# jchibane/Box2Mask

Hardware: AMD Instinct MI355X
Metric: ScanNet scenes/sec (fwd+bwd, ~150k voxels @2cm) (higher is better)
Workload: dtype f32; 1 GPU; ScanNet 2cm voxels, batch_size=8 per GPU, sparse-conv fwd/bwd + losses + Adam (BASELINE configs[1]); global_batch=8, ranks_seen=1, voxels_per_gpu_batch=1202778, parallelism=dp1, distinct_batches=4, setup_steps=2, prefetch=next batch: coordinate + kernel maps on a second stream during the step, steps_executed=51, full=False

## Files before the change

box2mask_amd/_lib.py:

```python
from __future__ import annotations

import ctypes as C
import os

import torch

_HERE = os.path.dirname(os.path.abspath(__file__))
LIB_PATH = os.environ.get('B2M_LIB_PATH', os.path.join(_HERE, 'libb2m_hip.so'))

P = C.c_void_p
I32 = C.c_int32
I64 = C.c_int64
F32 = C.c_float
F64 = C.c_double

PROTOTYPES = {
    'b2m_coords_build': [P, I64, P, P, I64, P, P],
    'b2m_morton_keys': [P, I64, P, P],
    'b2m_hilbert_keys': [P, I64, I32, P, P],
    'b2m_coords_stride': [P, I64, I32, P, P, P, P, P, I64, P, C.POINTER(I64), P],
    'b2m_kernel_map': [P, I64, I32, I32, P, P, I64, P, I32, I32, I32, P, I64, P],
    'b2m_occupancy': [P, I64, I32, I32, I32, I32, P, I64, P],
    'b2m_kernel_map_rulebook': [P, I64, I32, I32, P, P, I64, P, I32, I32, I32, P, P, P, P],
    'b2m_stride_tables': [P, P, I64, I64, P, I64, P, I64, P],
    'b2m_rulebook': [P, I64, I32, I64, P, P, P, P, P],
    'b2m_rulebook_balance': [P, I32, I64, P],
    'b2m_detection_loss': [P, I64, P, I64, P, I64, P, I64, I32, P, P, P, P, P, I64, F64, P, F32, F32, F32, F32, F32, P, P, P, P, P, P, P, P],
    'b2m_radix_argsort': [P, I64, C.c_uint64, P, P, P, P],
    'b2m_conv_fwd': [P, I64, I32, P, I64, I32, I64, P, I32, P, P, P, P, I64, P, I64, I32, I32, P],
    'b2m_conv_fwd_affine': [P, I64, I32, P, I64, I32, I64, P, I32, P, P, P, I64, P, I64, I32, P, P, P, I64, I32, P, P],
    'b2m_conv_fwd_h': [P, I64, I32, P, I64, I32, I64, P, I32, P, P, P, I64, P, I64, I32, P, P, P, I64, I32, P],
    'b2m_conv_fwd_h_stats': [P, I64, I32, P, I64, I32, I64, P, I32, P, P, P, I64, P, I64, I32, P, P],
    'b2m_weight_pack_h': [P, I64, I32, I32, I32, I32, P, P],
    'b2m_conv_fwd_stats': [P, I64, I32, P, I64, I32, I64, P, I32, P, P, P, P, I64, P, I64, I32, I32, P, P, P],
    'b2m_conv_wgrad_h': [P, I64, I32, I64, P, I64, I32, P, P, P, I64, I32, P, I64, I64, I32, F32, P],
    'b2m_weight_pack_h_t': [P, I32, I32, I32, I32, I32, I32, P, P],
    'b2m_bn_stats_finalize_h': [P, I64, I64, I32, P, P, P, F32, F32, P, P, P, P, P, P, P],
    'b2m_bn_stats_h': [P, I64, I64, I32, P, P, P],
    'b2m_bn_apply_h': [P, I64, I64, I32, P, P, P, I64, I32, P, I64, P],
    'b2m_bn_bwd_reduce_h': [P, I64, P, I64, P, I64, I64, I32, P, P, I32, P, P, P, P, P, P, F32, P],
    'b2m_bn_bwd_apply_h': [P, I64, P, I64, P, I64, I64, I32, P, P, P, P, F64, P, I32, P, P, P, I64, P, I64, P],
    'b2m_half_absmax': [P, I64, I64, I32, P, P],
    'b2m_f32_absmax': [P, I64, P, P],
    'b2m_guard_finish': [P, P, P, P],
    'b2m_clock_probe': [P, I32, P],
    'b2m_xchg_allreduce': [P, I32, P, I32, I32, C.c_uint64, P, P, P],
    'b2m_conv_up': [P, I64, I32, P, I64, I32, I64, P, I32, P, P, P, P, P, I64, I32, I64, I32, P, P, P, I64, I32, P, P],
    'b2m_weight_pack': [P, I64, I32, I32, I32, I32, I32, I32, I32, P, P],
    'b2m_weight_pack_run': [P, I32, I64, P],
    'b2m_weight_pack_h_run': [P, I32, I64, P],
    'b2m_conv_wgrad': [P, I64, I32, I64, P, I64, I32, P, P, P, I64, I32, P, I64, I64, P, P],
    'b2m_conv_wgrad_tr': [P, I64, I32, I64, P, I64, I32, P, P, P, I64, I32, P, I64, I64, P, P],
    'b2m_bn_stats': [P, I64, I64, I32, P, P, P],
    'b2m_bn_tilestats': [P, I64, I32, P, P, P],
    'b2m_bn_tilestats_finalize': [P, I64, I64, I32, P, P, P, P, F32, F32, P, P, P, P, P, P, P],
    'b2m_bn_finalize': [P, F64, P, I32, P, P, F32, F32, P, P, P, P, P, P, P],
    'b2m_bn_apply': [P, I64, I64, I32, P, P, P, I64, I32, P, I64, P],
    'b2m_bn_bwd_reduce': [P, I64, P, I64, P, I64, I64, I32, P, P, I32, P, P, P, P, P, P, P],
    'b2m_bn_stats_finalize': [P, I64, I64, I32, P, P, P, P, F32, F32, P, P, P, P, P, P, P],
    'b2m_bn_bwd_apply': [P, I64, P, I64, P, I64, I64, I32, P, P, P, P, F64, P, I32, P, P, P, I64, P, I64, P],
    'b2m_bn_apply2': [P, I64, P, I64, I64, I32, P, P, P, P, I32, P, I64, P],
    'b2m_bn_bwd_reduce2': [P, I64, P, I64, P, I64, P, I64, I64, I32, P, P, P, P, I32, P, P, P],
    'b2m_bn_bwd_apply2': [P, I64, P, I64, P, I64, P, I64, I64, I32, P, P, P, P, P, P, P, F64, P, I32, P, I64, P, I64, P, P, P, P, P, P],
    'b2m_bn_small_fwd': [P, I64, I64, I32, P, P, F32, F32, P, P, P, P, P, P, P, I64, I32, P, I64, P],
    'b2m_bn_small_fwd_stats': [P, I64, I64, I32, P, P],
    'b2m_bn_small_fwd_apply': [P, P, I64, I64, I32, P, P, F32, F32, P, P, P, P, P, P, P, I64, I32, P, I64, P],
    'b2m_bn_small_bwd_phase': [I32, P, I64, P, I64, P, I64, I64, I32, P, P, P, I32, P, P, P, P, P, I64, P, I64, P, P, P],
    'b2m_bn_small_bwd': [P, I64, P, I64, P, I64, I64, I32, P, P, P, I32, P, P, P, P, P, I64, P, I64, P],
    'b2m_relu_fwd': [P, I64, P, P],
    'b2m_relu_bwd': [P, P, I64, P, P],
    'b2m_add': [P, P, I64, P, P],
    'b2m_segment_pool_fwd': [P, I64, I64, I32, P, I64, I32, P, P, P, P, P],
    'b2m_segment_mean_sorted': [P, I64, I64, I32, P, P, I64, P, P, P],
    'b2m_segment_pool_bwd': [P, I64, I32, P, I64, I32, P, P, P, I64, P],
    'b2m_nmc': [P, I32, F32, I32, P, P, P, P, P, P],
    'b2m_nmc_batch': [P, P, I32, I32, F32, P, P, P, P, P, P],
    'b2m_mask_project': [P, I32, P, I32, P, P, I64, F32, P, I64, P],
    'b2m_mask_nms': [P, I32, I64, F32, P, P, P, P],
    'b2m_label_hist': [P, I64, P, I32, P, I64, I32, P, P],
    'b2m_mask_gather': [P, I64, P, I32, P, I64, P, P],
    'b2m_mask_project_batch': [P, I32, I64, I64, F32, P],
    'b2m_mask_nms_batch': [P, I32, I32, F32, P],
    'b2m_label_hist_batch': [P, I32, I64, I32, P],
    'b2m_mask_gather_batch': [P, I32, I64, I64, P],
    'b2m_mask_gather_batch_t': [P, I32, I64, I64, I64, P, P],
    'b2m_mask_nms_sweep': [P, I32, I64, P, I32, P, P, P],
    'b2m_mask_nms_sweep_batch': [P, I32, I32, P, I32, P, I64, P],
    'b2m_mask_hist_index': [P, I64, I32, I64, P, P, I64, I32, P, P, P],
    'b2m_mask_hist_index_batch': [P, I32, I64, I64, P],
    'b2m_mask_hist': [P, I64, I32, P, I64, I32, P, P],
    'b2m_mask_pack': [P, I32, I64, P, I64, P],
    'b2m_set_ious': [P, P, I64, P, P],
    'b2m_mask_hulls': [P, I64, I32, P, I64, P, P, P, I32, P, P, P, P, P, P, P],
    'b2m_mask_hulls_index': [P, I64, I32, I64, P, P, I64, P, P, P, P, I32, P, P, P, P, P, P, P],
    'b2m_mask_hulls_index_batch': [P, I32, I32, I32, I64, P],
    'b2m_obb_corners': [P, P, P, I32, P, P],
    'b2m_hull_box_iou': [P, P, P, P, I32, P, P, I32, P, P],
    'b2m_aabb_iou': [P, P, I32, P, P, P, I32, P, P],
    'b2m_dbscan': [P, I64, I32, F64, I32, P, P, P, P],
    'b2m_paint_proposals': [P, I64, I32, P, I64, I32, F64, I32, P, P, P, P, P],
    'b2m_joint_hist': [P, P, I64, I32, I32, P, P],
    'b2m_vox_shift': [P, I64, P, P, P],
    'b2m_unique_insert_async': [P, I64, P, I64, P, P, P, P],
    'b2m_vox_keys': [P, I64, P, F64, P, P, P],
    'b2m_sort_u64': [P, I64, P],
    'b2m_unique_rank': [P, I64, P, P, I64, P, I64, P, P],
    'b2m_vox_decode': [P, I64, I32, P, P],
    'b2m_vox_nearest': [P, I64, P, F64, P, P, I64, I64, P, P, P],
    'b2m_vox_gather': [P, I64, P, P, P, P, P, P],
    'b2m_seg_centroid': [P, P, I64, I64, F64, P, P, P, P, P],
    'b2m_box_membership': [P, I64, P, P, P, I32, P, P, P, P],
    'b2m_seg_box_vote': [P, I64, P, P, I64, I64, P, P, P, P, I32, P, P, P, P, P],
    'b2m_obb_membership': [P, I64, P, P, P, I32, P, P, P],
# ... 123 lines not shown
```

box2mask_amd/csrc/conv.hip:

```cpp
#include "b2m_common.h"
#include <stdlib.h>
#include <type_traits>

struct ConvArgs {
    const float* x1; int64_t ldx1; int c1;
    const float* x2; int64_t ldx2; int c2;
    const float* wp; int K;
    const float* bias;
    const int32_t* rb_in; const uint8_t* rb_out; const int32_t* rb_cnt;
    int64_t n_out, ntiles;
    float* y; int64_t ldy; int cout; int accumulate; int nstrips; int vec_store;
    int nslice;
    int chain;
    int fast32;
    const float* zeros;
    int ncs;
    int wg_combine;
    int64_t nwg;
    int64_t xcd_per;
    const int32_t* xcd_start;
    int64_t wg_per_tile;
    const int32_t* tile_order;
    double* stats;
    const float* ep_scale; const float* ep_shift; const float* ep_res; int64_t ld_res; int ep_relu;
// ... 508 lines not shown
        }
        bool more = true;
        while (more) {
#pragma unroll
            for (int u = 0; u < 3; ++u) {
                if (k0 < 0) { more = false; break; }
                const int n = count_of(k0);
                const int G = (n + 15) >> 4;
                const int k2c = valid(k2, valid(k1, k0)), k3c = valid(k3, k2c);
                load_ops(k2c, idx, av[(u + 2) % 3], w[(u + 2) % 3]);
                load_idx(k3c, idx);
                f32x4 acc[NG][TW];
#pragma unroll
                for (int g = 0; g < NG; ++g) {
                    if (g < G) {
#pragma unroll
                        for (int t = 0; t < TW; ++t) {
                            f32x4 c = {0.f, 0.f, 0.f, 0.f};
                            c = __builtin_amdgcn_mfma_f32_16x16x4f32(av[u][g][0], w[u][t], c, 0, 0, 0);
                            acc[g][t] = __builtin_amdgcn_mfma_f32_16x16x4f32(av[u][g][1], w[u][2 + t], c, 0, 0, 0);
                        }
                    }
                }
#pragma unroll
                for (int g = 0; g < NG; ++g) {
                    if (g < G) {
                        int ad[4];
                        float old[4][TW];
#pragma unroll
                        for (int r = 0; r < 4; ++r) {
                            ad[r] = (16 * g + 4 * q + r < n) ? (int)((out[u][g] >> (8 * r)) & 255) : B2M_TILE;
#pragma unroll
                            for (int t = 0; t < TW; ++t) old[r][t] = Cs[cs_index<TW>(ad[r], 16 * t + i)];
                        }
#pragma unroll
                        for (int r = 0; r < 4; ++r)
#pragma unroll
                            for (int t = 0; t < TW; ++t) Cs[cs_index<TW>(ad[r], 16 * t + i)] = old[r][t] + acc[g][t][r];
                    }
                }
                load_out(k3c, out[u]);
                k0 = k1; k1 = k2; k2 = k3;
                k3 = k2 < 0 ? -1 : next_active(k2);
            }
        }
        __builtin_amdgcn_fence(__ATOMIC_SEQ_CST, "wavefront");
    }
    if (a.stats && lane < a.cout) {
        const int64_t rem = a.n_out - row0;
        const int rows = rem < B2M_TILE ? (int)rem : B2M_TILE;
        double s1[4] = {0., 0., 0., 0.}, s2[4] = {0., 0., 0., 0.};
        int r = 0;
        for (; r + 3 < rows; r += 4) {
#pragma unroll
            for (int u = 0; u < 4; ++u) {
                const double v = (double)Cs[cs_index<TW>(r + u, lane)];
                s1[u] += v; s2[u] = fma(v, v, s2[u]);
            }
        }
        for (; r < rows; ++r) {
            const double v = (double)Cs[cs_index<TW>(r, lane)];
            s1[0] += v; s2[0] = fma(v, v, s2[0]);
        }
        double* o = a.stats + tile * 2 * a.cout + lane;
        o[0] = (s1[0] + s1[1]) + (s1[2] + s1[3]); o[a.cout] = (s2[0] + s2[1]) + (s2[2] + s2[3]);
    }
    for (int e = lane; e < B2M_TILE * (SW / 4); e += 64) {
        const int row = e / (SW / 4), c4 = (e % (SW / 4)) * 4;
        const int64_t grow = row0 + row;
        if (grow >= a.n_out) continue;
        f32x4 v = *(const f32x4*)&Cs[cs_index<TW>(row, c4)];
        float* dst = a.y + grow * a.ldy + c4;
        if (a.vec_store && c4 + 3 < a.cout) {
            if constexpr (EP) v = conv_epilogue(a, v, grow, c4);
            *(f32x4*)dst = v;
        } else {
#pragma unroll
            for (int u = 0; u < 4; ++u) if (c4 + u < a.cout) dst[u] = v[u];
        }
    }
}

#include "conv_fwd_flow.h"
#include "conv_1x1.h"

static inline int conv_kc(int cin) { return cin >= 16 ? 16 : 8; }
static inline int conv_tw(int cout, int K) { return (cout % 48 == 0 && K > 1 && b2m_env_int("B2M_CONV_TW3", 1)) ? 3 : 2; }

extern "C" int64_t b2m_weight_pack_size(int32_t K, int32_t cin, int32_t cout) {
    const int KC = conv_kc(cin);
    const int TW = conv_tw(cout, K);
    const int64_t nchunk = (cin + KC - 1) / KC, nstrip = (cout + 16 * TW - 1) / (16 * TW);
    return (int64_t)K * nstrip * nchunk * (64 * TW * (KC / 4));
}

__global__ void weight_pack_kernel(const float* __restrict__ w, int64_t ldw, int K, int rows, int cols, int transpose,
                                   int mirror, int sb, int CI, int CO, int KC, int TW, float* __restrict__ wp) {
    const int KS = KC / 4, LW = 64 * TW * KS, SW = 16 * TW;
    const int nchunk = (CI + KC - 1) / KC, nstrip = (CO + SW - 1) / SW;
    const int64_t total = (int64_t)K * nstrip * nchunk * LW;
    for (int64_t e = (int64_t)blockIdx.x * blockDim.x + threadIdx.x; e < total; e += (int64_t)gridDim.x * blockDim.x) {
        int lane, f;
        pack_unpos((int)(e % LW), TW * KS, lane, f);
        const int64_t blk = e / LW;
        const int chunk = (int)(blk % nchunk); const int64_t b2 = blk / nchunk;
        const int strip = (int)(b2 % nstrip); const int k = (int)(b2 / nstrip);
        const int s = f / TW, t = f % TW, q = lane >> 4, i = lane & 15;
        const int ci = chunk * KC + KS * q + s, co = strip * SW + 16 * t + i;
        float v = 0.f;
        if (ci < CI && co < CO) {
            if (!transpose) v = w[((int64_t)k * rows + ci) * ldw + co];
            else v = w[((int64_t)(mirror ? K - 1 - k : k) * rows + sb + co) * ldw + ci];
        }
        wp[e] = v;
    }
}
extern "C" int b2m_weight_pack(const float* w, int64_t ldw, int32_t K, int32_t cin, int32_t cout, int32_t transpose,
                               int32_t mirror, int32_t slice_begin, int32_t slice_count, float* wp, void* stream) {
    hipStream_t st = (hipStream_t)stream;
    B2M_CHECK_ARG(w && wp && K >= 1 && cin > 0 && cout > 0 && ldw >= cout, "bad arguments");
    int CI, CO;
    if (!transpose) { CI = cin; CO = cout; }
    else {
        B2M_CHECK_ARG(slice_begin >= 0 && slice_count > 0 && slice_begin + slice_count <= cin, "bad channel slice");
        CI = cout; CO = slice_count;
    }
    const int64_t total = b2m_weight_pack_size(K, CI, CO);
    int64_t grid = (total + 255) / 256;
    if (grid > 65536) grid = 65536;
    weight_pack_kernel<<<(unsigned)grid, 256, 0, st>>>(w, ldw, K, cin, cout, transpose, mirror, slice_begin, CI, CO,
                                                       conv_kc(CI), conv_tw(CO, K), wp);
    B2M_LAUNCH_CHECK();
    return B2M_OK;
}

struct PackDesc {
    const float* w; float* wp;
    int64_t ldw, first_block, total;
    int32_t K, rows, cols, transpose, mirror, sb, CI, CO, KC, TW;
};
extern "C" int32_t b2m_weight_pack_plan_size(void) { return (int32_t)sizeof(PackDesc); }
extern "C" int64_t b2m_weight_pack_plan(int32_t n, const int64_t* w, const int64_t* wp, const int64_t* ldw,
                                        const int32_t* K, const int32_t* cin, const int32_t* cout,
                                        const int32_t* transpose, const int32_t* mirror, const int32_t* slice_begin,
                                        const int32_t* slice_count, void* plan_host) {
    B2M_CHECK_ARG(n >= 0 && (n == 0 || (w && wp && ldw && K && cin && cout && transpose && mirror && slice_begin &&
                                        slice_count && plan_host)), "bad arguments");
    PackDesc* d = (PackDesc*)plan_host;
    int64_t blocks = 0;
    for (int i = 0; i < n; ++i) {
        B2M_CHECK_ARG(w[i] && wp[i] && K[i] >= 1 && cin[i] > 0 && cout[i] > 0 && ldw[i] >= cout[i], "bad layer");
        PackDesc e;
        e.w = (const float*)(uintptr_t)w[i]; e.wp = (float*)(uintptr_t)wp[i]; e.ldw = ldw[i];
        e.K = K[i]; e.rows = cin[i]; e.cols = cout[i]; e.transpose = transpose[i]; e.mirror = mirror[i]; e.sb = slice_begin[i];
        if (!transpose[i]) { e.CI = cin[i]; e.CO = cout[i]; }
        else {
            B2M_CHECK_ARG(slice_begin[i] >= 0 && slice_count[i] > 0 && slice_begin[i] + slice_count[i] <= cin[i], "bad channel slice");
            e.CI = cout[i]; e.CO = slice_count[i];
        }
        e.KC = conv_kc(e.CI); e.TW = conv_tw(e.CO, e.K);
        e.total = b2m_weight_pack_size(e.K, e.CI, e.CO);
        e.first_block = blocks;
        blocks += e.total / (64 * e.TW * (e.KC / 4));
        d[i] = e;
    }
    return blocks;
// ... 41 lines not shown
            float v = 0.f;
            if (ci0 + ci_l < d.CI && co0 + co_l < d.CO) {
                if (!d.transpose) v = d.w[((int64_t)k * d.rows + ci0 + ci_l) * d.ldw + co0 + co_l];
                else v = d.w[((int64_t)(d.mirror ? d.K - 1 - k : k) * d.rows + d.sb + co0 + co_l) * d.ldw + ci0 + ci_l];
            }
            tile[ci_l * SW + co_l] = v;
        }
    }
    __syncthreads();
    float* out = d.wp + pb * LW;
    if (KCc == 16) {
        const int e4 = threadIdx.x;
        if (e4 < LW / 4) {
            const int lane = e4 & 63, u = e4 >> 6, q = lane >> 4, i = lane & 15;
            f32x4 v;
#pragma unroll
            for (int r = 0; r < 4; ++r) {
                const int f = 4 * u + r, s_ = f / TW, t = f % TW;
                v[r] = tile[(KS * q + s_) * SW + 16 * t + i];
            }
            *(f32x4*)&out[4 * e4] = v;
        }
    } else {
        for (int e = threadIdx.x; e < LW; e += 256) {
            int lane, f;
            pack_unpos(e, TW * KS, lane, f);
            const int s_ = f / TW, t = f % TW, q = lane >> 4, i = lane & 15;
            out[e] = tile[(KS * q + s_) * SW + 16 * t + i];
        }
    }
}
__global__ __launch_bounds__(256) void weight_pack_batch_kernel(const PackDesc* __restrict__ plan, int n) {
    __shared__ __attribute__((aligned(16))) float tile[16 * 48];
    const int64_t blk0 = (int64_t)blockIdx.x * PACK_PER_WG;
    int lo = 0, hi = n - 1;
    while (lo < hi) {
        const int mid = (lo + hi + 1) >> 1;
        if (plan[mid].first_block <= blk0) lo = mid; else hi = mid - 1;
    }
    for (int it = 0; it < PACK_PER_WG; ++it) {
        const int64_t blk = blk0 + it;
        while (lo + 1 < n && plan[lo + 1].first_block <= blk) ++lo;
        const PackDesc d = plan[lo];
        const int64_t pb = blk - d.first_block;
        if (pb * (64 * d.TW * (d.KC / 4)) >= d.total) return;
        if (d.KC == 16 && d.TW == 3) pack_one_block<16, 3>(d, pb, tile);
        else if (d.KC == 16 && d.TW == 2) pack_one_block<16, 2>(d, pb, tile);
        else pack_one_block<0, 0>(d, pb, tile);
    }
}
extern "C" int b2m_weight_pack_run(const void* plan_dev, int32_t n, int64_t total_blocks, void* stream) {
    B2M_CHECK_ARG(n >= 0 && total_blocks >= 0 && total_blocks < (1ll << 31) && (n == 0 || plan_dev), "bad arguments");
    if (n == 0 || total_blocks == 0) return B2M_OK;
    weight_pack_batch_kernel<<<(unsigned)cdiv64(total_blocks, PACK_PER_WG), 256, 0, (hipStream_t)stream>>>((const PackDesc*)plan_dev, n);
    B2M_LAUNCH_CHECK();
    return B2M_OK;
}

static inline bool addr32(int64_t rows, int64_t ld, int esz) {
    return rows < (1 << 24) && ld < (1 << 22) && rows * ld * esz < (1ll << 32);
}
static inline bool addr32(int64_t rows, int64_t ld1, int64_t ld2, int esz) { return addr32(rows, ld1, esz) && addr32(rows, ld2, esz); }
static inline ConvArgs conv_args(const float* x1, int64_t ldx1, int c1, const float* x2, int64_t ldx2, int c2, const float* wp, int K,
                                 const int32_t* rb_in, const uint8_t* rb_out, const int32_t* rb_cnt, int64_t n_out, float* y, int64_t ldy,
                                 int cout, int TW) {
    ConvArgs a{};
    a.x1 = x1; a.ldx1 = ldx1; a.c1 = c1; a.x2 = x2; a.ldx2 = ldx2; a.c2 = c2;
    a.wp = wp; a.K = K;
    a.rb_in = rb_in; a.rb_out = rb_out; a.rb_cnt = rb_cnt;
    a.n_out = n_out; a.ntiles = cdiv64(n_out, B2M_TILE);
    a.y = y; a.ldy = ldy; a.cout = cout;
    a.nstrips = (cout + 16 * TW - 1) / (16 * TW);
    return a;
}
static inline unsigned conv_xcd_plan(ConvArgs& a, int64_t items_per_tile, int wpb, bool balanced) {
    const int64_t xcd_tiles = b2m_env_int("B2M_XCD", 1) ? (1 << 30) : 0;
    const XcdOrder o = xcd_order(a.nwg, xcd_tiles * items_per_tile / wpb);
    a.xcd_per = o.chunk;
    if (!(balanced && a.ntiles >= B2M_BALANCE_MIN_TILES && xcd_tiles > 0 && b2m_env_int("B2M_XCD_BALANCE", 1))) return o.grid;
    a.xcd_start = a.rb_cnt + (int64_t)a.K * a.ntiles;
    a.tile_order = b2m_env_int("B2M_XCD_ORDER", 1) ? a.xcd_start + 16 + a.ntiles : nullptr;
    a.wg_per_tile = items_per_tile / wpb;
    return (unsigned)(8 * B2M_XCD_CAP(a.ntiles) * a.wg_per_tile);
}

struct ConvEpilogue { const float* scale; const float* shift; const float* res; int64_t ld_res; int relu; };
static int conv_fwd_impl(const float* x1, int64_t ldx1, int32_t c1, const float* x2, int64_t ldx2, int32_t c2,
                         int64_t n_in, const float* wp, int32_t K, const float* bias, const int32_t* rb_in,
                         const uint8_t* rb_out, const int32_t* rb_cnt, int64_t n_out, float* y, int64_t ldy,
                         int32_t cout, int32_t accumulate, double* tile_stats, int32_t* wrote_stats, void* stream,
                         const ConvEpilogue* ep = nullptr, int32_t* fused = nullptr) {
    hipStream_t st = (hipStream_t)stream;
    if (wrote_stats) *wrote_stats = 0;
    if (fused) *fused = 0;
    B2M_CHECK_ARG(c1 > 0 && c2 >= 0 && cout > 0 && K >= 1 && K <= 128 && n_in >= 0 && n_out >= 0, "bad sizes (K<=128)");
    B2M_CHECK_ARG(ldy >= cout && ldx1 >= c1 && (c2 == 0 || ldx2 >= c2), "leading dimension too small");
    const int cin = c1 + c2;
    const int KC = conv_kc(cin);
    const int KS = KC / 4;
    B2M_CHECK_ARG(c2 == 0 || c1 % KC == 0, "with two sources c1 must be a multiple of 16");
    if (n_out == 0) return B2M_OK;
    B2M_CHECK_ARG(n_in >= 1, "n_in (rows of x1/x2) must be >= 1 where there are output rows");
    B2M_CHECK_ARG(x1 && wp && y, "bad pointers");
    B2M_CHECK_ARG((rb_in == nullptr) == (rb_out == nullptr) && (rb_in == nullptr) == (rb_cnt == nullptr),
                  "rulebook pointers must be all set or all NULL");
    B2M_CHECK_ARG(rb_in != nullptr || K == 1, "identity rulebook needs K == 1");
    B2M_CHECK_ARG(c2 == 0 || x2 != nullptr, "x2 is NULL");
    B2M_CHECK_ARG(((uintptr_t)wp % 16) == 0, "packed weights must be 16-byte aligned");
    const bool fast = c1 % KC == 0 && c2 % KC == 0 && ldx1 % KS == 0 && (c2 == 0 || ldx2 % KS == 0) &&
                      ((uintptr_t)x1 % (4 * KS)) == 0 && ((uintptr_t)x2 % (4 * KS)) == 0;
    const int TW = conv_tw(cout, K);
    ConvArgs a = conv_args(x1, ldx1, c1, x2, ldx2, c2, wp, K, rb_in, rb_out, rb_cnt, n_out, y, ldy, cout, TW);
    a.bias = bias; a.accumulate = accumulate;
    a.vec_store = (ldy % 4 == 0 && ((uintptr_t)y % 16) == 0) ? 1 : 0;
    const bool ep_ok = ep && ep->scale && ep->shift && a.vec_store && cout % 4 == 0 && !accumulate && !bias &&
                       ((uintptr_t)ep->scale % 16) == 0 && ((uintptr_t)ep->shift % 16) == 0 &&
                       (!ep->res || (ep->ld_res % 4 == 0 && ep->ld_res >= cout && ((uintptr_t)ep->res % 16) == 0));
    auto use_epilogue = [&]() {
        a.ep_scale = ep->scale; a.ep_shift = ep->shift; a.ep_res = ep->res; a.ld_res = ep->ld_res; a.ep_relu = ep->relu;
        if (fused) *fused = 1;
    };
    const int64_t items0 = a.ntiles * a.nstrips;
    int nslice = 1;
    const int64_t target = b2m_env_int("B2M_DETERMINISTIC", 0) ? 0 : b2m_env_int("B2M_CONV_TARGET", cin <= 32 ? 4096 : 6144);
    if (items0 < target && K > 1) {
        nslice = (int)cdiv64(target, items0);
        if (nslice > 16) nslice = 16;
        if (nslice > K) nslice = K;
        if (K >= 4 && nslice > 1) {
            nslice = (nslice + 3) / 4 * 4;
            if (nslice > K) nslice = K / 4 * 4;
            if (nslice > 16) nslice = 16;
            const int cap = b2m_env_int("B2M_CONV_MAXSLICE", a.ntiles >= 8 ? 4 : 16);
            if (nslice > cap) nslice = cap;
        }
    }
    int ncs = 1;
    const int nchunk_h = (cin + KC - 1) / KC;
    while (nslice > 1 && ncs < 4 && items0 * nslice * ncs < b2m_env_int("B2M_CONV_CHUNK_ITEMS", 2048) && nchunk_h / (ncs * 2) >= 2 &&
           b2m_env_int("B2M_CONV_CHUNKSPLIT", 1)) ncs *= 2;
    nslice *= ncs;
    a.fast32 = (addr32(n_in, ldx1, ldx2, 4) && b2m_env_int("B2M_CONV_FAST32", 1)) ? 1 : 0;
    bool split2 = false;
    if (nslice == 1 && K >= 8 && rb_in != nullptr && fast && KC == 16 && a.fast32 && (cin / 16) % 2 == 0 && cin >= 32 &&
        b2m_env_int("B2M_CONV_PIPE", 2) && b2m_env_int("B2M_CONV_HANDLOADS", 1) && !b2m_env_int("B2M_PIPE_DBG", 0) &&
        !b2m_env_int("B2M_DETERMINISTIC", 0) && items0 >= target && items0 < b2m_env_int("B2M_CONV_SPLIT2", 0)) {
        nslice = 2;
        split2 = true;
    }
    a.ncs = ncs;
    a.nslice = nslice;
    a.wg_combine = ((nslice > 1 && nslice % 4 == 0 && b2m_env_int("B2M_CONV_WGCOMBINE", 1)) || split2) ? 1 : 0;
    static const float* zeros_addr = nullptr;
    if (!zeros_addr) B2M_HIP(hipGetSymbolAddress((void**)&zeros_addr, HIP_SYMBOL(g_zeros)));
    a.zeros = zeros_addr;
    if (nslice > 1 && !accumulate && !(a.wg_combine && (nslice == 4 || split2)))
        B2M_HIP(hipMemset2DAsync(y, (size_t)ldy * sizeof(float), 0, (size_t)cout * sizeof(float), (size_t)n_out, st));
    const int64_t items = items0 * nslice;
    a.nwg = cdiv64(items, 4);
    const unsigned grid = conv_xcd_plan(a, (int64_t)a.nstrips * nslice, 4, false);
    const bool ident = rb_in == nullptr;
    if (ident && fast && KC == 16 && a.fast32 && n_in >= n_out && b2m_env_int("B2M_CONV_1X1", 1)) {
        int spw = a.nstrips % 3 == 0 ? 3 : a.nstrips % 2 == 0 ? 2 : 1;
        if (a.ntiles * (a.nstrips / spw) < 2048) spw = 1;
        const int64_t g1 = a.ntiles * (a.nstrips / spw);
        B2M_CHECK_ARG(g1 < (1ll << 31), "too many workgroups");
        if (ep_ok) use_epilogue();
        if (spw == 3) conv_1x1_kernel<3><<<(unsigned)g1, 64, 0, st>>>(a);
        else if (spw == 2) conv_1x1_kernel<2><<<(unsigned)g1, 64, 0, st>>>(a);
        else conv_1x1_kernel<1><<<(unsigned)g1, 64, 0, st>>>(a);
        B2M_LAUNCH_CHECK();
        return B2M_OK;
    }
    {
        const int nc = cin / 16;
        const int depth = b2m_env_int("B2M_CONV_PIPE", 2) ? 2 : 0;
        const bool split_ok = nslice == 1 || (a.wg_combine && b2m_env_int("B2M_CONV_FLOW_SPLIT", 1));
        if (depth >= 2 && !ident && fast && KC == 16 && split_ok && a.fast32 && nc % ncs == 0 && (nc / ncs) % depth == 0 &&
            nc / ncs >= depth) {
            const int wpb = nslice == 1 ? 1 : split2 ? 2 : 4;
            B2M_CHECK_ARG(items0 < (1ll << 31), "too many (tile, strip) items");
            a.chain = (wpb == 1 && b2m_env_int("B2M_CONV_CHAIN", 1)) ? 1 : 0;
            if (tile_stats && (nslice == 1 || ((nslice == 4 || split2) && !accumulate))) {
                a.stats = tile_stats;
                if (wrote_stats) *wrote_stats = 1;
            }
            if (ep_ok && (nslice == 1 || nslice == 4 || split2)) use_epilogue();
            a.nwg = cdiv64(items, wpb);
            const unsigned fgrid = conv_xcd_plan(a, (int64_t)a.nstrips * nslice, wpb, (a.nstrips * nslice) % wpb == 0);
            const int dbg = b2m_env_int("B2M_PIPE_DBG", 0);
            const int hl = b2m_env_int("B2M_CONV_HANDLOADS", 1);
            if (hl && depth == 2 && dbg == 32 && wpb == 1 && TW == 3) {
                conv_fwd_flow_kernel<2, 3, 32, 1, 1><<<fgrid, 64, 0, st>>>(a);
                B2M_LAUNCH_CHECK();
                return B2M_OK;
            }
            if (hl && depth == 2 && dbg == 8 && wpb == 1 && TW == 3) {
                conv_fwd_flow_kernel<2, 3, 8, 1, 1><<<fgrid, 64, 0, st>>>(a);
                B2M_LAUNCH_CHECK();
                return B2M_OK;
            }
            if (hl && depth == 2 && !dbg) {
                if (wpb == 2) {
                    if (TW == 3) conv_fwd_flow_kernel<2, 3, 0, 2, 1><<<fgrid, 128, 0, st>>>(a);
                    else conv_fwd_flow_kernel<2, 2, 0, 2, 1><<<fgrid, 128, 0, st>>>(a);
                } else if (wpb == 4) {
                    if (TW == 3) conv_fwd_flow_kernel<2, 3, 0, 4, 1><<<fgrid, 256, 0, st>>>(a);
                    else conv_fwd_flow_kernel<2, 2, 0, 4, 1><<<fgrid, 256, 0, st>>>(a);
                } else {
                    if (TW == 3) conv_fwd_flow_kernel<2, 3, 0, 1, 1><<<fgrid, 64, 0, st>>>(a);
                    else conv_fwd_flow_kernel<2, 2, 0, 1, 1><<<fgrid, 64, 0, st>>>(a);
                }
                B2M_LAUNCH_CHECK();
                return B2M_OK;
            }
            if (wpb == 4) {
                if (TW == 3) conv_fwd_flow_kernel<2, 3, 0, 4><<<fgrid, 256, 0, st>>>(a);
                else conv_fwd_flow_kernel<2, 2, 0, 4><<<fgrid, 256, 0, st>>>(a);
            } else if (dbg && TW == 3) {
                switch (dbg) {
                    case 1: conv_fwd_flow_kernel<2, 3, 1><<<fgrid, 64, 0, st>>>(a); break;
                    case 2: conv_fwd_flow_kernel<2, 3, 2><<<fgrid, 64, 0, st>>>(a); break;
                    case 4: conv_fwd_flow_kernel<2, 3, 4><<<fgrid, 64, 0, st>>>(a); break;
                    case 8: conv_fwd_flow_kernel<2, 3, 8><<<fgrid, 64, 0, st>>>(a); break;
                    default: conv_fwd_flow_kernel<2, 3, 6><<<fgrid, 64, 0, st>>>(a); break;
                }
            } else {
                if (TW == 3) conv_fwd_flow_kernel<2, 3><<<fgrid, 64, 0, st>>>(a);
                else conv_fwd_flow_kernel<2, 2><<<fgrid, 64, 0, st>>>(a);
            }
            B2M_LAUNCH_CHECK();
            return B2M_OK;
        }
    }
    if (KC == 8 && !ident && fast && cin == 8 && c2 == 0 && nslice == 1 && a.nstrips == 1 && TW == 2 && a.fast32 &&
        b2m_env_int("B2M_CONV_STEM", 1)) {
        if (tile_stats) {
            a.stats = tile_stats;
            if (wrote_stats) *wrote_stats = 1;
        }
// ... 1244 lines not shown
```

include/b2m.h:

```cpp
#ifndef B2M_H
#define B2M_H
#include <stdint.h>
#ifdef __cplusplus
extern "C" {
#endif

#define B2M_TILE 64
#define B2M_OK 0
#define B2M_ERR_ARG (-1)
#define B2M_ERR_HIP (-2)
#define B2M_ERR_UNSUPPORTED (-3)

const char* b2m_last_error(void);
int b2m_version(void);
int b2m_device_ok(void);
int b2m_reload_env(void);


int b2m_coords_build(const int32_t* coords, int64_t n, uint64_t* keys, int32_t* vals, int64_t cap,
                     int32_t* dup_count, void* stream);

int b2m_morton_keys(const int32_t* coords, int64_t n, int64_t* keys, void* stream);
int b2m_hilbert_keys(const int32_t* coords, int64_t n, int32_t bits, int64_t* keys, void* stream);

int64_t b2m_radix_argsort_scratch(int64_t n);
int b2m_radix_argsort(const uint64_t* keys, int64_t n, uint64_t bit_mask, int64_t* perm, int64_t* inv_perm, void* scratch,
                      void* stream);

int b2m_coords_stride(const int32_t* coords, int64_t n, int32_t ts,
                      int32_t* coords_out, int32_t* parent, int32_t* koff,
                      uint64_t* keys, int32_t* vals, int64_t cap,
                      int32_t* scratch, int64_t* n_out_host, void* stream);

int b2m_kernel_map(const int32_t* coords, int64_t n, int32_t ksize, int32_t ts,
                   const uint64_t* keys, const int32_t* vals, int64_t cap,
                   const uint64_t* occ, int32_t dim_x, int32_t dim_y, int32_t dim_z,
                   int32_t* nbr, int64_t ld, void* stream);

int b2m_kernel_map_rulebook(const int32_t* coords, int64_t n, int32_t ksize, int32_t ts,
                            const uint64_t* keys, const int32_t* vals, int64_t cap,
                            const uint64_t* occ, int32_t dim_x, int32_t dim_y, int32_t dim_z,
                            int32_t* rb_in, uint8_t* rb_out, int32_t* rb_cnt, void* stream);

int b2m_occupancy(const int32_t* coords, int64_t n, int32_t batches, int32_t dim_x, int32_t dim_y, int32_t dim_z,
                  uint64_t* bits, int64_t words, void* stream);

int b2m_stride_tables(const int32_t* parent, const int32_t* koff, int64_t n_fine, int64_t n_coarse,
                      int32_t* child, int64_t ld_c, int32_t* up, int64_t ld_f, void* stream);

int64_t b2m_rulebook_cnt_size(int32_t K, int64_t n_out);
int b2m_rulebook_balance(int32_t* rb_cnt, int32_t K, int64_t n_out, void* stream);
int b2m_rulebook(const int32_t* nbr, int64_t ld, int32_t K, int64_t n_out,
                 int32_t* rb_in, uint8_t* rb_out, int32_t* rb_cnt, int32_t* pair_total, void* stream);

int b2m_detection_loss(const float* off, int64_t ld_off, const float* bnd, int64_t ld_bnd, const float* sc, int64_t ld_sc,
                       const float* sem, int64_t ld_sem, int32_t n_class, const float* gt_off, const float* gt_bnd,
                       const float* loc, const uint8_t* fg, const int64_t* gt_sem, int64_t S, double n_fg,
                       const double* n_valid, float w_off, float w_bnd, float w_sc, float w_sem, float min_bb_size,
                       float* d_off, float* d_bnd, float* d_sc, float* d_sem, int64_t* argmax, double* sums,
                       float* result, void* stream);


int64_t b2m_weight_pack_size(int32_t K, int32_t cin, int32_t cout);
int b2m_weight_pack(const float* w, int64_t ldw, int32_t K, int32_t cin, int32_t cout, int32_t transpose,
                    int32_t mirror, int32_t slice_begin, int32_t slice_count, float* wp, void* stream);

int32_t b2m_weight_pack_plan_size(void);
int64_t b2m_weight_pack_plan(int32_t n, const int64_t* w, const int64_t* wp, const int64_t* ldw, const int32_t* K,
                             const int32_t* cin, const int32_t* cout, const int32_t* transpose,
                             const int32_t* mirror, const int32_t* slice_begin, const int32_t* slice_count,
                             void* plan_host);
int b2m_weight_pack_run(const void* plan_dev, int32_t n, int64_t total_blocks, void* stream);

int b2m_conv_fwd(const float* x1, int64_t ldx1, int32_t c1, const float* x2, int64_t ldx2, int32_t c2,
                 int64_t n_in, const float* wp, int32_t K, const float* bias,
                 const int32_t* rb_in, const uint8_t* rb_out, const int32_t* rb_cnt,
                 int64_t n_out, float* y, int64_t ldy, int32_t cout, int32_t accumulate, void* stream);

int b2m_conv_fwd_stats(const float* x1, int64_t ldx1, int32_t c1, const float* x2, int64_t ldx2, int32_t c2,
                       int64_t n_in, const float* wp, int32_t K, const float* bias,
                       const int32_t* rb_in, const uint8_t* rb_out, const int32_t* rb_cnt,
                       int64_t n_out, float* y, int64_t ldy, int32_t cout, int32_t accumulate,
                       double* tile_stats, int32_t* wrote_stats, void* stream);

int b2m_conv_fwd_affine(const float* x1, int64_t ldx1, int32_t c1, const float* x2, int64_t ldx2, int32_t c2,
                        int64_t n_in, const float* wp, int32_t K,
                        const int32_t* rb_in, const uint8_t* rb_out, const int32_t* rb_cnt,
                        int64_t n_out, float* y, int64_t ldy, int32_t cout,
                        const float* scale, const float* shift, const float* res, int64_t ld_res, int32_t relu,
                        int32_t* fused, void* stream);

int64_t b2m_weight_pack_h_size(int32_t K, int32_t c1, int32_t c2, int32_t cout);
int b2m_weight_pack_h(const float* w, int64_t ldw, int32_t K, int32_t c1, int32_t c2, int32_t cout, void* wp, void* stream);
int b2m_conv_fwd_h(const void* x1, int64_t ldx1, int32_t c1, const void* x2, int64_t ldx2, int32_t c2, int64_t n_in,
                   const void* wp, int32_t K, const int32_t* rb_in, const uint8_t* rb_out, const int32_t* rb_cnt,
                   int64_t n_out, void* y, int64_t ldy, int32_t cout, const float* scale, const float* shift,
                   const void* res, int64_t ld_res, int32_t relu, void* stream);
int b2m_conv_fwd_h_stats(const void* x1, int64_t ldx1, int32_t c1, const void* x2, int64_t ldx2, int32_t c2, int64_t n_in,
                         const void* wp, int32_t K, const int32_t* rb_in, const uint8_t* rb_out, const int32_t* rb_cnt,
                         int64_t n_out, void* y, int64_t ldy, int32_t cout, double* tile_stats, void* stream);

int b2m_conv_up(const float* x1, int64_t ldx1, int32_t c1, const float* x2, int64_t ldx2, int32_t c2, int64_t n_coarse,
                const float* wp, int32_t K, const float* bias, const int32_t* rb_in, const uint8_t* rb_out,
                const int32_t* rb_cnt, float* y, int64_t ldy, int32_t cout, int64_t n_fine, int32_t accumulate,
                const float* scale, const float* shift, const float* res, int64_t ld_res, int32_t relu,
                int32_t* ran, void* stream);

int64_t b2m_conv_wgrad_workspace(int32_t K, int32_t cin, int32_t cout);
int b2m_conv_wgrad(const float* x, int64_t ldx, int32_t cin, int64_t n_in, const float* dy, int64_t lddy, int32_t cout,
                   const int32_t* rb_in, const uint8_t* rb_out, const int32_t* rb_cnt,
                   int64_t n_out, int32_t K, float* dw, int64_t lddw, int64_t dw_kstride, float* workspace, void* stream);
int b2m_conv_wgrad_tr(const float* x, int64_t ldx, int32_t cin, int64_t n_in, const float* dy, int64_t lddy, int32_t cout,
                   const int32_t* rb_in, const uint8_t* rb_out, const int32_t* rb_cnt,
                   int64_t n_out, int32_t K, float* dw, int64_t lddw, int64_t dw_kstride, float* workspace, void* stream);

int b2m_conv_wgrad_h(const void* x, int64_t ldx, int32_t cin, int64_t n_in, const void* dy, int64_t lddy, int32_t cout,
                     const int32_t* rb_in, const uint8_t* rb_out, const int32_t* rb_cnt, int64_t n_out, int32_t K,
                     float* dw, int64_t lddw, int64_t dw_kstride, int32_t tr, float out_scale, void* stream);
int b2m_weight_pack_h_t(const float* w, int32_t K, int32_t cin, int32_t cout, int32_t mirror, int32_t s0, int32_t sc, void* wp,
                        void* stream);
int32_t b2m_weight_pack_h_plan_size(void);
int64_t b2m_weight_pack_h_plan(int32_t n, const int64_t* w, const int64_t* wp, const int32_t* K, const int32_t* cin, const int32_t* cout,
                               const int32_t* c1, const int32_t* transposed, const int32_t* mirror, const int32_t* s0, const int32_t* sc,
                               void* plan_host);
int b2m_weight_pack_h_run(const void* plan_dev, int32_t n, int64_t total_blocks, void* stream);
int b2m_bn_stats_finalize_h(const void* x, int64_t ldx, int64_t n, int32_t c, double* partial, const float* gamma, const float* beta,
                            float eps, float momentum, float* running_mean, float* running_var, float* mean, float* invstd,
                            float* scale, float* shift, void* stream);
int b2m_bn_stats_h(const void* x, int64_t ldx, int64_t n, int32_t c, double* partial, double* stats, void* stream);
int b2m_bn_apply_h(const void* x, int64_t ldx, int64_t n, int32_t c, const float* scale, const float* shift,
                   const void* residual, int64_t ldr, int32_t relu, void* y, int64_t ldy, void* stream);
int b2m_bn_bwd_reduce_h(const void* dy, int64_t lddy, const void* y, int64_t ldy, const void* x, int64_t ldx, int64_t n,
                        int32_t c, const float* mean, const float* invstd, int32_t relu, const float* mask_scale,
                        const float* mask_shift, double* partial, double* sums,
                        float* dbeta_f32, float* dgamma_f32, float param_grad_scale, void* stream);
int b2m_bn_bwd_apply_h(const void* dy, int64_t lddy, const void* y, int64_t ldy, const void* x, int64_t ldx, int64_t n,
                       int32_t c, const float* mean, const float* invstd, const float* gamma, const double* sums,
                       double count, const double* count_dev, int32_t relu, const float* mask_scale, const float* mask_shift,
                       void* dx, int64_t lddx, void* dres, int64_t lddres, void* stream);

int b2m_half_absmax(const void* x, int64_t ld, int64_t n, int32_t c, uint32_t* out, void* stream);
int b2m_f32_absmax(const float* g, int64_t n, uint32_t* out, void* stream);
int b2m_guard_finish(const uint32_t* flags, float* found_inf, uint32_t* counters, void* stream);

int64_t b2m_xchg_size(void);
int32_t b2m_xchg_max_doubles(void);
int32_t b2m_xchg_max_ranks(void);
int b2m_xchg_alloc(void** buf, void* handle64);
int b2m_xchg_open(const void* handle64, void** ptr);
int b2m_xchg_close(void* ptr);
int b2m_xchg_free(void* buf);
int32_t b2m_xchg_is_finegrained(const void* buf);
int b2m_xchg_allreduce(const double* vals, int32_t n, const void* const* peers_dev, int32_t rank, int32_t world,
                       uint64_t epoch, double* out, int32_t* err, void* stream);

int b2m_clock_probe(unsigned long long* out4, int32_t iters, void* stream);


int b2m_bn_stats(const float* x, int64_t ldx, int64_t n, int32_t c, double* partial, double* stats, void* stream);

int b2m_bn_stats_finalize(const float* x, int64_t ldx, int64_t n, int32_t c, double* partial, double* stats,
                          const float* gamma, const float* beta, float eps, float momentum,
                          float* running_mean, float* running_var, float* mean, float* invstd,
                          float* scale, float* shift, void* stream);

int b2m_bn_tilestats(const double* tile_stats, int64_t ntiles, int32_t c, double* partial, double* stats, void* stream);
int b2m_bn_tilestats_finalize(const double* tile_stats, int64_t ntiles, int64_t n, int32_t c, double* partial,
                              double* stats, const float* gamma, const float* beta, float eps, float momentum,
                              float* running_mean, float* running_var, float* mean, float* invstd, float* scale,
                              float* shift, void* stream);

int b2m_bn_finalize(const double* stats, double count, const double* count_dev, int32_t c, const float* gamma, const float* beta,
                    float eps, float momentum, float* running_mean, float* running_var,
// ... 167 lines not shown
```

Baseline: 118.8 scenes/s.

## Add weight-stationary sparse conv kernel for tiny coarse levels

Adds a weight-stationary forward conv kernel. It keeps a channel-slice of one kernel offset's weights in registers and streams the rulebook pairs through MFMA, scattering results with atomicAdd. It is used when both input and output row counts are at most 256 (env-tunable) and the split-K path would otherwise run. The goal is to stop tiny deep-level convolutions from reloading weights per tile and wasting most of the grid on nearly empty tiles. In exchange it adds float atomics (non-deterministic summation order) and a debug launch counter.

```diff
diff --git a/box2mask_amd/_lib.py b/box2mask_amd/_lib.py
--- a/box2mask_amd/_lib.py
+++ b/box2mask_amd/_lib.py
@@ -29,6 +29,7 @@
     'b2m_radix_argsort': [P, I64, C.c_uint64, P, P, P, P],
     'b2m_conv_fwd': [P, I64, I32, P, I64, I32, I64, P, I32, P, P, P, P, I64, P, I64, I32, I32, P],
     'b2m_conv_fwd_affine': [P, I64, I32, P, I64, I32, I64, P, I32, P, P, P, I64, P, I64, I32, P, P, P, I64, I32, P, P],
+    'b2m_debug_ws_launches': [I32],
     'b2m_conv_fwd_h': [P, I64, I32, P, I64, I32, I64, P, I32, P, P, P, I64, P, I64, I32, P, P, P, I64, I32, P],
     'b2m_conv_fwd_h_stats': [P, I64, I32, P, I64, I32, I64, P, I32, P, P, P, I64, P, I64, I32, P, P],
     'b2m_weight_pack_h': [P, I64, I32, I32, I32, I32, P, P],
diff --git a/box2mask_amd/csrc/conv.hip b/box2mask_amd/csrc/conv.hip
--- a/box2mask_amd/csrc/conv.hip
+++ b/box2mask_amd/csrc/conv.hip
@@ -614,6 +614,7 @@
 }
 
 #include "conv_fwd_flow.h"
+#include "conv_ws.h"
 #include "conv_1x1.h"
 
 static inline int conv_kc(int cin) { return cin >= 16 ? 16 : 8; }
@@ -821,6 +822,11 @@
     a.tile_order = b2m_env_int("B2M_XCD_ORDER", 1) ? a.xcd_start + 16 + a.ntiles : nullptr;
     a.wg_per_tile = items_per_tile / wpb;
     return (unsigned)(8 * B2M_XCD_CAP(a.ntiles) * a.wg_per_tile);
+}
+
+static int g_ws_launches = 0;
+extern "C" int b2m_debug_ws_launches(int32_t reset) {
+    return reset ? __atomic_exchange_n(&g_ws_launches, 0, __ATOMIC_RELAXED) : __atomic_load_n(&g_ws_launches, __ATOMIC_RELAXED);
 }
 
 struct ConvEpilogue { const float* scale; const float* shift; const float* res; int64_t ld_res; int relu; };
@@ -895,6 +901,24 @@
     a.zeros = zeros_addr;
     if (nslice > 1 && !accumulate && !(a.wg_combine && (nslice == 4 || split2)))
         B2M_HIP(hipMemset2DAsync(y, (size_t)ldy * sizeof(float), 0, (size_t)cout * sizeof(float), (size_t)n_out, st));
+    if (nslice > 1 && !(a.wg_combine && (nslice == 4 || split2)) && rb_in != nullptr && K > 1 && fast && KC == 16 && a.fast32 && !bias &&
+        n_out <= b2m_env_int("B2M_CONV_WS_ROWS", 256) && n_in <= b2m_env_int("B2M_CONV_WS_ROWS", 256) && b2m_env_int("B2M_CONV_WS", 1)) {
+        ConvWsArgs s{};
+        s.x1 = x1; s.x2 = x2; s.ld1 = (uint32_t)ldx1 * 4u; s.ld2 = c2 ? (uint32_t)ldx2 * 4u : 0u;
+        s.nch1 = c1 / 16; s.nch = cin / 16;
+        s.wp = wp; s.rb_in = rb_in; s.rb_out = rb_out; s.rb_cnt = rb_cnt;
+        s.ntiles = (int)a.ntiles; s.nstrips = a.nstrips;
+        const int pcmax = TW == 3 ? 8 : 16;
+        s.nparts = (s.nch + pcmax - 1) / pcmax; s.pc = (s.nch + s.nparts - 1) / s.nparts;
+        s.y = y; s.ldy = ldy; s.cout = cout;
+        const unsigned wgrid = (unsigned)(K * s.nstrips * s.nparts);
+        const bool full = s.pc == pcmax && s.nch % pcmax == 0;
+        if (TW == 3) { if (full) conv_ws_kernel<3, true><<<wgrid, 256, 0, st>>>(s); else conv_ws_kernel<3, false><<<wgrid, 256, 0, st>>>(s); }
+        else { if (full) conv_ws_kernel<2, true><<<wgrid, 256, 0, st>>>(s); else conv_ws_kernel<2, false><<<wgrid, 256, 0, st>>>(s); }
+        B2M_LAUNCH_CHECK();
+        __atomic_fetch_add(&g_ws_launches, 1, __ATOMIC_RELAXED);
+        return B2M_OK;
+    }
     const int64_t items = items0 * nslice;
     a.nwg = cdiv64(items, 4);
     const unsigned grid = conv_xcd_plan(a, (int64_t)a.nstrips * nslice, 4, false);
diff --git a/box2mask_amd/csrc/conv_ws.h b/box2mask_amd/csrc/conv_ws.h
--- /dev/null
+++ b/box2mask_amd/csrc/conv_ws.h
@@ -0,0 +1,157 @@
+#pragma once
+
+struct ConvWsArgs {
+    const float* x1; const float* x2;
+    uint32_t ld1, ld2;
+    int nch1, nch;
+    const float* wp;
+    const int32_t* rb_in; const uint8_t* rb_out; const int32_t* rb_cnt;
+    int ntiles, nstrips;
+    int nparts, pc;
+    float* y; int64_t ldy; int cout;
+};
+
+template <int TW, bool FULL>
+__global__ __launch_bounds__(256, 1) void conv_ws_kernel(ConvWsArgs a) {
+    constexpr int PC = TW == 2 ? 16 : 8;
+    constexpr int SW = 16 * TW;
+    constexpr int LW = 64 * TW * 4;
+    const int lane = threadIdx.x & 63;
+    const int wave = __builtin_amdgcn_readfirstlane(threadIdx.x >> 6);
+    const int i = lane & 15, q = lane >> 4;
+    const uint32_t item = blockIdx.x;
+    const int part = (int)(item % (uint32_t)a.nparts);
+    const uint32_t ks = item / (uint32_t)a.nparts;
+    const int strip = (int)(ks % (uint32_t)a.nstrips);
+    const int k = (int)(ks / (uint32_t)a.nstrips);
+    const int cb = part * a.pc;
+    const int npc = FULL ? PC : (a.nch - cb < a.pc ? a.nch - cb : a.pc);
+    if (!FULL && npc <= 0) return;
+    const int ntiles = a.ntiles;
+    const int32_t* cntp = a.rb_cnt + (int64_t)k * ntiles;
+
+    int w_tb = 0, w_base = 0, w_cntv = 0, w_tile = 0, w_cnt = 0, w_g = 0, w_G = 0, w_pos = 0;
+    uint64_t w_act = 0;
+    auto next_visit = [&](int& tile, int& g, int& cnt) -> bool {
+        for (;;) {
+            while (w_g < w_G) {
+                const int gg = w_g++;
+                if (((w_pos++) & 3) == wave) { tile = w_tile; g = gg; cnt = w_cnt; return true; }
+            }
+            while (!w_act) {
+                if (w_tb >= ntiles) return false;
+                w_cntv = w_tb + lane < ntiles ? cntp[w_tb + lane] : 0;
+                w_act = __ballot(w_cntv > 0);
+                w_base = w_tb; w_tb += 64;
+            }
+            const int tl = __builtin_ctzll(w_act);
+            w_act &= w_act - 1;
+            w_cnt = __builtin_amdgcn_readlane(w_cntv, tl);
+            w_tile = w_base + tl; w_g = 0; w_G = (w_cnt + 15) >> 4;
+        }
+    };
+    int t0, g0, n0;
+    if (!next_visit(t0, g0, n0)) return;
+
+    f32x4 W[PC][TW];
+    {
+        const float* wsrc = a.wp + ((size_t)((uint32_t)k * (uint32_t)a.nstrips + (uint32_t)strip) * (uint32_t)a.nch + (uint32_t)cb) * LW + lane * 4;
+#pragma unroll
+        for (int c = 0; c < PC; ++c) {
+#pragma unroll
+            for (int u = 0; u < TW; ++u) W[c][u] = f32x4{0.f, 0.f, 0.f, 0.f};
+            if (FULL || c < npc) {
+#pragma unroll
+                for (int u = 0; u < TW; ++u) W[c][u] = *(const f32x4*)(wsrc + c * LW + u * 256);
+            }
+        }
+    }
+#define B2M_WS_W(c, s, t) W[c][(TW * (s) + (t)) >> 2][(TW * (s) + (t)) & 3]
+
+    const int64_t ldr = (int64_t)ntiles * B2M_TILE;
+    const int32_t* rin_k = a.rb_in + (int64_t)k * ldr;
+    const uint8_t* rout_k = a.rb_out + (int64_t)k * ldr;
+    const uint32_t q16 = (uint32_t)q * 16u;
+    const int col0 = strip * SW;
+
+    auto pair_load = [&](int tile, int g, int cnt, int& r_in, int& r_out) {
+        const int j = 16 * g + i;
+        r_in = -1; r_out = 0;
+        if (j < cnt) {
+            const int64_t e = (int64_t)tile * B2M_TILE + j;
+            r_in = rin_k[e];
+            r_out = rout_k[e];
+        }
+    };
+    auto gather = [&](f32x4 (&xv)[PC], int r_in) {
+#pragma unroll
+        for (int c = 0; c < PC; ++c) xv[c] = f32x4{0.f, 0.f, 0.f, 0.f};
+        if (r_in >= 0) {
+            const uint32_t off1 = __umul24((uint32_t)r_in, a.ld1) + q16, off2 = __umul24((uint32_t)r_in, a.ld2) + q16;
+#pragma unroll
+            for (int c = 0; c < PC; ++c) {
+                if (FULL || c < npc) {
+                    const int cg = cb + c;
+                    const bool first = cg < a.nch1;
+                    const char* src = first ? (const char*)a.x1 + (size_t)cg * 64 : (const char*)a.x2 + (size_t)(cg - a.nch1) * 64;
+                    xv[c] = *(const f32x4*)(src + (first ? off1 : off2));
+                }
+            }
+        }
+    };
+    auto step = [&](const f32x4 (&xc)[PC], f32x4 (&xn)[PC], int tile, int r_in, int r_out, bool more, int r_in_next) {
+        f32x4 acc[2][TW];
+#pragma unroll
+        for (int h = 0; h < 2; ++h)
+#pragma unroll
+            for (int t = 0; t < TW; ++t) acc[h][t] = f32x4{0.f, 0.f, 0.f, 0.f};
+        auto mfmas = [&](int c) {
+#pragma unroll
+            for (int s = 0; s < 4; ++s)
+#pragma unroll
+                for (int t = 0; t < TW; ++t)
+                    acc[c & 1][t] = __builtin_amdgcn_mfma_f32_16x16x4f32(xc[c][s], B2M_WS_W(c, s, t), acc[c & 1][t], 0, 0, 0);
+        };
+        mfmas(0);
+        if (more) gather(xn, r_in_next);
+#pragma unroll
+        for (int c = 1; c < PC; ++c)
+            if (FULL || c < npc) mfmas(c);
+        __builtin_amdgcn_sched_barrier(0);
+        __builtin_amdgcn_s_waitcnt(0x0F70);
+        __builtin_amdgcn_sched_barrier(0);
+        const int enc = r_in >= 0 ? r_out : -1;
+#pragma unroll
+        for (int r = 0; r < 4; ++r) {
+            const int orow = __builtin_amdgcn_ds_bpermute((4 * q + r) << 2, enc);
+            if (orow >= 0) {
+                float* dst = a.y + ((int64_t)tile * B2M_TILE + orow) * a.ldy + col0 + i;
+#pragma unroll
+                for (int t = 0; t < TW; ++t)
+                    if (col0 + 16 * t + i < a.cout) atomicAdd(dst + 16 * t, acc[0][t][r] + acc[1][t][r]);
+            }
+        }
+    };
+
+    f32x4 xa[PC], xb[PC];
+    int ia, oa, ib = -1, ob = 0, ic = -1, oc = 0;
+    int t1 = 0, g1, n1, t2 = 0, g2, n2;
+    pair_load(t0, g0, n0, ia, oa);
+    bool v1 = next_visit(t1, g1, n1);
+    if (v1) pair_load(t1, g1, n1, ib, ob);
+    gather(xa, ia);
+    __builtin_amdgcn_s_waitcnt(0x0F70);
+    for (;;) {
+        const bool v2 = v1 && next_visit(t2, g2, n2);
+        if (v2) pair_load(t2, g2, n2, ic, oc);
+        step(xa, xb, t0, ia, oa, v1, ib);
+        if (!v1) break;
+        v1 = v2 && next_visit(t0, g0, n0);
+        if (v1) pair_load(t0, g0, n0, ia, oa);
+        step(xb, xa, t1, ib, ob, v2, ic);
+        if (!v2) break;
+        { const int tt = t2; t2 = t1; t1 = t0; t0 = tt; }
+        { const int ti = ic, to = oc; ic = ib; oc = ob; ib = ia; ob = oa; ia = ti; oa = to; }
+    }
+#undef B2M_WS_W
+}
diff --git a/include/b2m.h b/include/b2m.h
--- a/include/b2m.h
+++ b/include/b2m.h
@@ -89,6 +89,8 @@
                         int64_t n_out, float* y, int64_t ldy, int32_t cout,
                         const float* scale, const float* shift, const float* res, int64_t ld_res, int32_t relu,
                         int32_t* fused, void* stream);
+
+int b2m_debug_ws_launches(int32_t reset);
 
 int64_t b2m_weight_pack_h_size(int32_t K, int32_t c1, int32_t c2, int32_t cout);
 int b2m_weight_pack_h(const float* w, int64_t ldw, int32_t K, int32_t c1, int32_t c2, int32_t cout, void* wp, void* stream);
```

Result: no change. 118.7 scenes/s (-0.1%).
